# masa-ue/SVDD

Hardware: AMD Instinct MI355X
Metric: decoded sequences/sec (whole node), L=200 M=10 128-step SVDD-MC (higher is better)
Workload: dtype f32; 1 GPU; DNA enhancer SVDD-MC, batch=256/GPU, L=200, M=10, 128 steps (BASELINE.json configs[1]); dilated-CNN backbone 3.3M params + ConvGRU value net; global_batch=256, rng=philox

## Files before the change

include/svdd_hip.h:

```cpp
#ifndef SVDD_HIP_H
#define SVDD_HIP_H

#include <stdint.h>

#ifdef __cplusplus
extern "C" {
#endif

#define SVDD_VOCAB 5
#define SVDD_MASK 4
#define SVDD_MAX_M 1024

enum {
  SVDD_OK = 0,
  SVDD_E_ARG = -1,
  SVDD_E_LAUNCH = -2,
  SVDD_E_NODEVICE = -3
};

enum {
  SVDD_LAYOUT_BLV = 0,
  SVDD_LAYOUT_BVL = 1
};

// ... 99 lines not shown
int svdd_bb_layer_bwd_f32(const float* g_hn, const float* f_in, const float* tb, const float* gamma, float eps, const float* g_in,
                          const uint8_t* mask_prev, float* g_out, float* gt_out, int64_t rows, int rows_per_seq, int channels,
                          void* stream);
int svdd_gru_bidir_train_f32(const float* x, const float* wpack, const float* bpack, float* out, float* save, int n, int L,
                             void* stream);
int svdd_gru_bidir_bwd_f32(const float* grad_out, const float* out, const float* save, const float* wpack_bwd, float* dx, int n,
                           int L, void* stream);
int svdd_value_tail_f32(const float* h_fwd, const float* h_bwd, const float* w1pack, const float* b1,
                        const float* w_eff, const float* b_eff, float* out, int n, int L, int n_tasks,
                        const int32_t* count, void* stream);
int svdd_gru_set_mode(int mode);

int svdd_epilogue_ln_f32(const float* y, const float* bias, const float* f_prev, const float* tb,
                         const float* gamma, const float* beta, float* f_out, float* hn, int64_t rows,
                         int channels, int act, void* stream);

int svdd_conv1d_cl_f32(const float* x, const float* wpack, float* y, int n, int L, int cin, int cout,
                       int taps, int dilation, const float* bias, const float* f_prev, int act,
                       const float* tb, const float* gamma, const float* beta, float* hn, void* stream);
int svdd_conv1d_set_dynamic(int on);

int svdd_conv_tower_f32(const float* onehot, const float* tiles, const float* bias, float* out, int n, int L,
                        int nlayers, int residual_mask, const int32_t* count, void* stream);

int svdd_set_backbone_packing(int full);

int svdd_set_tower_version(int v);

int svdd_candidate_windows(const uint8_t* cand, const uint8_t* x, int B, int L, int M, int margin, int32_t* win,
                           int32_t* flags, void* stream);
int svdd_conv_tower_windows_f32(const float* onehot, const float* tiles, const float* bias, const int32_t* win,
                                const float* parent_out, float* out, int n, int L, int M, int nlayers,
                                int residual_mask, const int32_t* live_idx, const int32_t* count, void* stream);

int svdd_backbone_cnn_f32(const uint8_t* x, const float* table0, const float* tiles, const float* vec,
                          const float* w2, float* out, int n, int L, int nlayers, const int* dilations,
                          const int32_t* count, const int32_t* row_idx, int out_scatter, void* stream);
int svdd_backbone_cnn_save_f32(const uint8_t* x, const float* table0, const float* tiles, const float* vec, const float* w2,
                               float* out, int n, int L, int nlayers, const int* dilations, float* xhat, float* rstd,
                               unsigned long long* mask, void* stream);
int svdd_backbone_cnn_grad_f32(const float* dlogits, const float* tiles_bwd, const float* gamma, const float* w2,
                               const float* table0, const float* xhat, const float* rstd, const unsigned long long* mask,
                               float* dx, int n, int L, int nlayers, const int* dilations, void* stream);
int svdd_backbone_incr_f32(const uint8_t* x, const float* table0, const float* tiles, const float* vec, const float* w2,
                           float* out, int n, int L, int nlayers, const int* dilations, int lead, float* planes,
                           uint8_t* x_prev, int32_t* items, unsigned long long* stat, int first, int max_item, void* on_stream);
int svdd_backbone_incr2_f32(const uint8_t* x, const float* table0, const float* tiles, const float* vec, const float* w2,
                            float* out, int n, int L, int nlayers, const int* dilations, int lead, float* planes,
                            uint8_t* x_prev, int32_t* items, unsigned long long* stat, int first, int max_item,
                            int32_t* order, int32_t* order_count, void* on_stream);
int svdd_backbone_incr_set_residency(int wg_per_cu);
int svdd_backbone_set_workspace(void* ws, long long bytes);
int svdd_backbone_split_status(int* err);

enum { SVDD_PREC_F32 = 0, SVDD_PREC_F16X3 = 1, SVDD_PREC_BF16X3 = 2, SVDD_PREC_F16 = 3, SVDD_PREC_BF16 = 4 };

int svdd_backbone_cnn_lp(const uint8_t* x, const float* table0, const void* tiles, const float* vec,
                         const float* lscale, const float* w2, float* out, int n, int L, int nlayers,
                         const int* dilations, int prec, const int32_t* count, const int32_t* row_idx, int out_scatter,
                         void* stream);

int svdd_conv_tower_lp(const uint8_t* tok, const void* tiles, const float* bias, const float* inv, void* out,
                       int n, int L, int nlayers, int residual_mask, const int32_t* count, int prec, void* stream);
int svdd_conv_tower_windows_lp(const uint8_t* cand, const void* tiles, const float* bias, const float* inv,
                               const int32_t* win, const void* parent_out, void* out, int n, int L, int M,
                               int nlayers, int residual_mask, const int32_t* live_idx, const int32_t* count,
// ... 77 lines not shown
```

svdd_amd/_lib.py:

```python
import ctypes
import os
import subprocess

_HERE = os.path.dirname(os.path.abspath(__file__))
CSRC = os.path.join(_HERE, "csrc")
SO_PATH = os.environ.get("SVDD_HIP_LIB") or os.path.join(CSRC, "libsvdd_hip.so")
ABI_VERSION = 17

OK, E_ARG, E_LAUNCH, E_NODEVICE = 0, -1, -2, -3
LAYOUT_BLV, LAYOUT_BVL = 0, 1
RNG_REPLAY, RNG_PHILOX = 0, 1
SELECT_ARGMAX, SELECT_MULTINOMIAL = 0, 1
TARGET_MEAN, TARGET_LOGMEANEXP = 0, 1
EVOLVE_GLOBAL, EVOLVE_ROW = 0, 1
ATTR_GRADIENT, ATTR_TIMES_INPUT = 0, 1
PRECISIONS = {"f32": 0, "f16x3": 1, "bf16x3": 2, "f16": 3, "bf16": 4}
MAX_M = 1024

OPT_FORCE_EXACT, OPT_MSPLIT, OPT_SELECT_ONE_ROW, OPT_BACKBONE_LP_VERSION, OPT_TRUNK_GEMM_VERSION = 0, 1, 2, 3, 4
OPT_CAND_ROW_STRIDE, OPT_TRUNK_PLANES_F32, OPT_BACKBONE_SPLIT, OPT_SELECT_BATCHES = 5, 6, 7, 8


class SvddRng(ctypes.Structure):
    _fields_ = [("kind", ctypes.c_int32), ("step", ctypes.c_uint32), ("uniforms", ctypes.c_void_p),
# ... 62 lines not shown
    "svdd_trunk_attn_pool": (vp, vp, i32, i32, i32, vp, vp, vp, vp, vp, vp, i32, STREAM),
    "svdd_trunk_stem_unfold": (vp, i32, i32, vp, vp, STREAM),
    "svdd_trunk_attn_small": (vp, vp, vp, vp, i32, i32, i32, i32, i32, vp, vp, vp, STREAM),
    "svdd_trunk_windows": (vp, vp, vp, i32, i32, i32, i32, i32, i32, vp, vp, vp, vp, STREAM),
    "svdd_trunk_stem_unfold_win": (vp, i32, i32, i32, vp, vp, vp, vp, vp, STREAM),
    "svdd_trunk_attn_pool_win": (vp, vp, i32, i32, i32, i32, i32, vp, vp, vp, vp, i32, vp, vp, vp, vp, vp, vp, vp, i32, vp, vp, vp, STREAM),
    "svdd_bb_layer_fwd_f32": (vp, vp, vp, vp, vp, vp, f32, vp, vp, vp, i64, i32, i32, STREAM),
    "svdd_bb_layer_bwd_f32": (vp, vp, vp, vp, f32, vp, vp, vp, vp, i64, i32, i32, STREAM),
    "svdd_mt19937_uniform_f32": (vp, vp, i64, STREAM),
    "svdd_backbone_set_workspace": (vp, i64),
    "svdd_backbone_split_status": (pi32,),
    "svdd_backbone_cnn_save_f32": (vp, vp, vp, vp, vp, vp, i32, i32, i32, pi32, vp, vp, vp, STREAM),
    "svdd_backbone_cnn_grad_f32": (vp, vp, vp, vp, vp, vp, vp, vp, vp, i32, i32, i32, pi32, STREAM),
    "svdd_dps_probs": (vp, vp, i32, i32, vp, STREAM),
    "svdd_dps_probs_bwd": (vp, vp, vp, i32, i32, vp, vp, STREAM),
    "svdd_dps_guided_q": (vp, vp, vp, vp, f32, f32, f32, i32, i32, vp, STREAM),
    "svdd_reward_stem_f32": (vp, vp, vp, vp, i32, i32, i32, STREAM),
    "svdd_reward_stem_bwd_f32": (vp, vp, vp, i32, i32, i32, STREAM),
    "svdd_conv1d_cl_gated_f32": (vp, vp, vp, i32, i32, i32, i32, i32, i32, vp, vp, STREAM),
    "svdd_reward_tail_grad_f32": (vp, vp, vp, vp, vp, vp, vp, f32, i32, i32, vp, vp, STREAM),
    "svdd_sum_gate_f32": (vp, vp, vp, vp, i64, STREAM),
    "svdd_gru_bidir_train2_f32": (vp, vp, vp, vp, vp, vp, i32, i32, STREAM),
    "svdd_gru_bidir_bwd2_f32": (vp, vp, vp, vp, vp, vp, vp, i32, i32, STREAM),
    "svdd_classifier_propose": (vp, i32, vp, vp, f32, f32, f32, i32, i32, RNG, vp, vp, vp, STREAM),
    "svdd_elbo_mask": (vp, i32, i32, i32, f64, RNG, vp, vp, vp, vp, vp, vp, STREAM),
    "svdd_elbo_nll": (vp, i32, vp, vp, vp, i32, i32, i32, vp, vp, vp, vp, STREAM),
    "svdd_refine_remask": (vp, vp, vp, vp, vp, f32, i32, i32, RNG, vp, vp, vp, vp, vp, vp, vp),
    "svdd_value_target": (vp, vp, i32, i32, i32, i32, f32, vp, vp, vp, vp),
    "svdd_ism_mutants": (vp, vp, vp, i32, i32, i32, vp, vp, vp, vp),
    "svdd_ism_fold": (vp, vp, vp, vp, vp, vp, i32, i32, i32, i32, i32, vp, vp, vp, vp, vp),
    "svdd_evolve_apply": (vp, vp, vp, i32, i32, i32, vp, vp, vp, vp, vp, vp, vp, vp, vp, vp, vp, vp),
    "svdd_attr_path": (vp, vp, i32, vp, i32, i32, i32, i32, i32, i32, vp, vp, vp),
    "svdd_attr_fold": (vp, f32, vp, vp, vp, i32, i32, i32, i32, i32, i32, i32, vp, vp, vp, vp),
}
EXPORTS = tuple(SIGNATURES)


def build(force=False):
    import glob
    srcs = sorted(glob.glob(os.path.join(CSRC, "*.hip")) + glob.glob(os.path.join(CSRC, "*.h")) + [os.path.join(CSRC, "Makefile")])
    srcs.append(os.path.join(os.path.dirname(_HERE), "include", "svdd_hip.h"))
    if os.environ.get("SVDD_HIP_LIB"):
        return SO_PATH
    stale = not os.path.exists(SO_PATH) or os.path.getmtime(SO_PATH) < max(os.path.getmtime(f) for f in srcs)
    if force or stale:
        subprocess.check_call(["make", "-C", CSRC, "-B", "-j", str(min(8, os.cpu_count() or 1))])
    return SO_PATH


_lib = None


def lib():
    global _lib
    if _lib is not None:
        return _lib
    import torch
    if not os.path.exists(SO_PATH):
        raise SvddError(f"{SO_PATH} is missing: build it with `python -c 'import __graft_entry__ as g; g.build()'` "
                        "or `make -C svdd_amd/csrc`. There is no CPU fallback for the SVDD hot path.")
    L = ctypes.CDLL(SO_PATH)
    for name in EXPORTS:
        if not hasattr(L, name):
            raise SvddError(f"libsvdd_hip.so does not export {name}")
    if L.svdd_abi_version() != ABI_VERSION:
        raise SvddError(f"libsvdd_hip.so ABI {L.svdd_abi_version()} != binding ABI {ABI_VERSION}; rebuild")
# ... 102 lines not shown
```

svdd_amd/csrc/svdd_nets.hip:

```cpp
#include "svdd_host.h"

namespace {

typedef float f32x4 __attribute__((ext_vector_type(4)));

__device__ __forceinline__ float wave_sum(float v) {
#pragma unroll
  for (int off = 32; off > 0; off >>= 1) v += __shfl_xor(v, off, 64);
  return v;
}


constexpr int H = 64;
constexpr int HPAD = H + 4;

__device__ __forceinline__ float sigmoid_fast(float a) {
  return __builtin_amdgcn_rcpf(1.0f + __builtin_amdgcn_exp2f(-1.44269504088896f * a));
}
__device__ __forceinline__ float tanh_fast(float a) {
  return 1.0f - 2.0f * __builtin_amdgcn_rcpf(1.0f + __builtin_amdgcn_exp2f(2.88539008177793f * a));
}

template <bool BOTH>
__global__ __launch_bounds__(BOTH ? 512 : 256) void gru_bidir_kernel(const float* __restrict__ x, const float* __restrict__ wpack,
// ... 1131 lines not shown
    }
  }
  for (int e = tid; e < (TW_ROWS + 2) * TW_AP; e += 512) smem[e] = 0.0f;

  TowerCtx2 c;
  c.act = act; c.xs = xs; c.bias = a.bias;
  c.L = L; c.tile_rows = tile_rows; c.nlayers = a.nlayers; c.residual_mask = a.residual_mask;
  constexpr int CG = 4 / CT, RS = 2 * CT;
  c.cp = w % CG; c.rq = w / CG; c.j = lane & 15; c.g = lane >> 4;
  c.wsrc = a.tiles + (16 * CT * c.cp + c.j) * CH + 8 * c.g;
#pragma unroll
  for (int r = 0; r < 7; ++r) {
    const int row = 16 * (c.rq + RS * r) + c.j;
    c.apos[r] = (!SPT1 && !WIN && row < tile_rows) ? row % L : -(1 << 20);
  }
  const int nlive = ((WIN ? nt : TW_ROWS / 16) - c.rq + RS - 1) / RS;
  __syncthreads();
  tower2_dispatch<SPT1 || WIN, WIN, CT>(c, nlive);
  if (WIN) {
    for (int e = tid; e < L * 16; e += 512) {
      const int row = e >> 4, q = e & 15;
      if (row >= keep_lo && row < keep_hi)
        *reinterpret_cast<float4*>(outc + (size_t)row * TW_C + 4 * q) = *reinterpret_cast<const float4*>(act + (row - w0) * TW_AP + 4 * q);
    }
  } else {
    for (int e = tid; e < tile_rows * 16; e += 512) {
      const int row = e >> 4, q = e & 15;
      if (row0 + row < total_rows)
        *reinterpret_cast<float4*>(a.out + (row0 + row) * TW_C + 4 * q) = *reinterpret_cast<const float4*>(act + row * TW_AP + 4 * q);
    }
  }
}

__global__ __launch_bounds__(256) void candidate_windows_kernel(const uint8_t* __restrict__ cand, const uint8_t* __restrict__ x,
                                                               int n, int L, int M, int margin, int* __restrict__ win,
                                                               int* __restrict__ flags) {
  const int c = blockIdx.x * 4 + (threadIdx.x >> 6);
  if (c >= n) return;
  const int lane = threadIdx.x & 63;
  const uint8_t* cp = cand + (size_t)c * L;
  const uint8_t* xp = x + (size_t)(c / M) * L;
  int lo = 1 << 30, hi = -1;
  for (int l = lane; l < L; l += 64)
    if (cp[l] != xp[l]) { lo = min(lo, l); hi = max(hi, l); }
#pragma unroll
  for (int off = 32; off > 0; off >>= 1) { lo = min(lo, __shfl_xor(lo, off, 64)); hi = max(hi, __shfl_xor(hi, off, 64)); }
  if (lane == 0) {
    int w0 = 0, w1 = 0;
    if (hi >= 0) {
      w0 = max(0, lo - margin) & ~15;
      w1 = min((L + 15) & ~15, (hi + margin + 1 + 15) & ~15);
    }
    win[2 * c] = w0; win[2 * c + 1] = w1;
    if (flags) flags[c] = (w1 - w0) >> 4;
  }
}


struct BackboneArgs {
  const uint8_t* x;
  const float* table0;
  const float* tiles;
  const float* vec;
  const float* w2;
  float* out;
  int n, L, spt, nl;
  int dil[BB_MAXL];
  const int* count;
  const int* row_idx;
  int out_scatter;
  int auto_spt, ncu;
  SvddTilePlan plan;
  float* planes;
  int planes_P;
};

struct BackboneSave {
  float* xhat;
  float* rstd;
  unsigned long long* mask;
};

// ... 560 lines not shown
  int* toks = reinterpret_cast<int*>(rstat + ROWS);

  int item, seq;
  if (ORD) {
    if ((int)blockIdx.x >= a.order_count[a.layer - 1]) return;
    const unsigned ent = (unsigned)__builtin_amdgcn_readfirstlane(a.order[(size_t)(a.layer - 1) * a.order_stride + blockIdx.x]);
    item = (int)(ent & 0xFFFFu);
    seq = (int)(ent >> 16);
  } else {
    item = __builtin_amdgcn_readfirstlane(a.items[(size_t)(a.layer - 1) * a.n * SEG_SLOTS + blockIdx.x]);
    seq = blockIdx.x / SEG_SLOTS;
  }
  const int nown = min(item >> 8, NC);
  if (nown == 0) return;
  const int t0 = item & 255;
  const int tid = threadIdx.x, lane = tid & 63;
  const int cg = __builtin_amdgcn_readfirstlane(tid >> 6);
  const int j = lane & 15, g = lane >> 4;
  const int col0 = 32 * cg + j;
  const int L = a.L;
  const int r0 = 16 * (t0 - 1);
  const size_t pl_stride = (size_t)a.n * TW_ROWS * BB_C;
  float* pl0 = a.planes + (size_t)seq * TW_ROWS * BB_C;
  const int cl = a.layer - 1;
#define SEG_LIVE(S) ((S) <= nown + 1)

  f32x4 f[NS][2], acc[NS][2];
  if (a.layer == 1) {
    for (int e = tid; e < ROWS + 8; e += 256) {
      const int p = r0 - 4 + e;
      toks[e] = (p >= 0 && p < L) ? (int)a.x[(size_t)seq * L + p] : -1;
    }
    __syncthreads();
#pragma unroll
    for (int ct = 0; ct < 2; ++ct) {
      const int col = col0 + 16 * ct;
      const float b0 = a.vec[col];
#pragma unroll
      for (int s = 0; s < NS; ++s) {
        if (!SEG_LIVE(s)) continue;
#pragma unroll
        for (int e = 0; e < 4; ++e) {
          const int ri = 16 * s + 4 * g + e, row = r0 + ri;
          float v = b0;
#pragma unroll
          for (int t = 0; t < 9; ++t) {
            const int tk = toks[ri + t];
            if (tk >= 0) v += a.table0[(t * 5 + tk) * BB_C + col];
          }
          f[s][ct][e] = (row >= 0 && row < L) ? fmaxf(v, 0.0f) : 0.0f;
        }
      }
    }
  } else {
    const float* src = pl0 + (size_t)(a.layer - 2) * pl_stride;
#pragma unroll
    for (int s = 0; s < NS; ++s) {
      if (!SEG_LIVE(s)) continue;
#pragma unroll
      for (int ct = 0; ct < 2; ++ct)
#pragma unroll
        for (int e = 0; e < 4; ++e) {
          const int row = r0 + 16 * s + 4 * g + e;
          f[s][ct][e] = (row >= 0 && row < L) ? src[row * BB_C + col0 + 16 * ct] : 0.0f;
        }
    }
  }

  const float* vl = a.vec + (size_t)(cl + 1) * 4 * BB_C;
  {
    const float tb0 = vl[BB_C + col0], tb1 = vl[BB_C + col0 + 16];
#pragma unroll
    for (int s = 0; s < NS; ++s) {
      if (!SEG_LIVE(s)) continue;
#pragma unroll
      for (int e = 0; e < 4; ++e) {
        const float sm = group16_sum((f[s][0][e] + tb0) + (f[s][1][e] + tb1));
        if (j == 0) psum[cg * ROWS + 16 * s + 4 * g + e] = sm;
      }
    }
    __syncthreads();
    if (tid < 16 * (nown + 2))
      rstat[tid] = ((psum[tid] + psum[ROWS + tid]) + (psum[2 * ROWS + tid] + psum[3 * ROWS + tid])) * (1.0f / BB_C);
    __syncthreads();
#pragma unroll
// ... 1136 lines not shown
  void (*seg)(BackboneSegArgs) = max_item == 4 ? backbone_seg_kernel<4, true> : max_item == 2 ? backbone_seg_kernel<2, true>
                                                                                                : backbone_seg_kernel<1, true>;
  svdd_raise_lds_limit(seg, slds);
  for (int k = 1; k <= lead; ++k) {
    sa.layer = k;
    if (svdd_launch(seg, sgrid, dim3(256), slds, stream, sa) != SVDD_OK) return SVDD_E_LAUNCH;
  }
  return svdd_launch_timed(span.last(), backbone_kernel<true, false, 2>, dim3((unsigned)n), dim3(512), lds, stream, a, BackboneSave{});
}

typedef decltype(&value_tail_kernel<1>) ValueTailKernel;

extern "C" int svdd_value_tail_f32(const float* h_fwd, const float* h_bwd, const float* w1pack, const float* b1,
                                   const float* w_eff, const float* b_eff, float* out, int n, int L, int n_tasks,
                                   const int32_t* count, void* stream) {
  if (!h_fwd || !h_bwd || !w1pack || !b1 || !w_eff || !b_eff || !out || n <= 0 || L <= 0 || n_tasks < 1 || n_tasks > 4)
    return SVDD_E_ARG;
  ValueTailKernel kern;
  switch (n_tasks) {
    case 1: kern = value_tail_kernel<1>; break;
    case 2: kern = value_tail_kernel<2>; break;
    case 3: kern = value_tail_kernel<3>; break;
    default: kern = value_tail_kernel<4>; break;
  }
  SvddSpan span(SVDD_SLOT_VALUE_TAIL);
  return svdd_launch_timed(span.all(), kern, dim3((unsigned)((n + 3) / 4)), dim3(256), 0, stream, h_fwd, h_bwd, w1pack, b1, w_eff, b_eff, out,
                           n, L, count);
}

extern "C" int svdd_candidate_windows(const uint8_t* cand, const uint8_t* x, int B, int L, int M, int margin, int32_t* win,
                                      int32_t* flags, void* stream) {
  if (!cand || !x || !win || B <= 0 || L <= 0 || M <= 0 || margin < 0) return SVDD_E_ARG;
  const int n = B * M;
  return svdd_launch(candidate_windows_kernel, dim3((unsigned)((n + 3) / 4)), dim3(256), 0, stream, cand, x, n, L, M, margin, win, flags);
}

extern "C" int svdd_conv_tower_windows_f32(const float* onehot, const float* tiles, const float* bias, const int32_t* win,
                                           const float* parent_out, float* out, int n, int L, int M, int nlayers,
                                           int residual_mask, const int32_t* live_idx, const int32_t* count, void* stream) {
  if (!onehot || !tiles || !bias || !win || !parent_out || !out || n <= 0 || M <= 0 || (n % M && !live_idx) || L <= TW_ROWS / 2 ||
      L > TW_ROWS || nlayers != 5)
    return SVDD_E_ARG;
  TowerWinArgs wa{TowerArgs{onehot, tiles, bias, out, n, L, 1, nlayers, residual_mask, nullptr}, win, parent_out, M, live_idx, count};
  void (*kern)(TowerWinArgs) = conv_tower_win_kernel;
  if (g_tower_ver != 1) kern = g_tower_ver == 2 ? conv_tower2_kernel<true, true, 2> : conv_tower2_kernel<true, true, 1>;
  SvddSpan span(SVDD_SLOT_CONV_TOWER);
  return svdd_launch_timed(span.all(), kern, dim3((unsigned)n), dim3(512), svdd_lds_raised(tower2_lds_bytes()), stream, wa);
}
```

svdd_amd/diffusion.py:

```python
import contextlib
import functools
import math
import warnings
import weakref
from dataclasses import dataclass
from typing import Optional

import numpy as np
import torch
import torch.nn.functional as F
from torch import nn

from . import noise_schedule, ops
from .backbone import CNNModel


@dataclass
class Loss:
    loss: torch.Tensor
    nlls: torch.Tensor
    token_mask: torch.Tensor


@dataclass
# ... 1030 lines not shown
        pos, pos_dev = self._ism_positions(positions, x.shape[1])
        if chunk_rows is not None and int(chunk_rows) <= 0:
            raise ValueError(f"chunk_rows must be positive, got {chunk_rows}")
        if not x.dtype.is_floating_point and x.dtype != torch.bool and bool((x == self.mask_index).any()):
            raise ops.SvddError("x holds a MASK token: in-silico mutagenesis scores finished sequences (tokens 0..3)")
        x_u8, _ = self._refine_inputs(x, None)
        self._require_gpu()
        B, L = x_u8.shape
        if chunk_rows is None:
            chunk_rows = self.ISM_WAVES_PER_CHUNK * torch.cuda.get_device_properties(self.device).multi_processor_count
        Pc = max(1, min(len(pos), int(chunk_rows) // (3 * B)))
        return x_u8, pos_dev, len(pos), Pc

    class _IsmWorkspace:
        def __init__(self, B, L, Pc, dev, windowed):
            n = B * 3 * Pc
            self.cand = torch.empty(n * L, dtype=torch.uint8, device=dev)
            self.onehot = self.flags = self.live_idx = self.slot = self.count = None
            if windowed:
                self.onehot = torch.empty(n * L * 4, dtype=torch.float32, device=dev)
                self.flags, self.live_idx, self.slot = (torch.empty(n, dtype=torch.int32, device=dev) for _ in range(3))
                self.count = torch.zeros(1, dtype=torch.int32, device=dev)
            self.err = torch.zeros(1, dtype=torch.int32, device=dev)

    def _ism_route(self, pre_scorer_embedding, pre_scorer_head, reward_model, L):
        from .fused import FusedValueNet
        score_fn = self._design_scorer(pre_scorer_embedding, pre_scorer_head, reward_model)
        fn = (self.value_callable(pre_scorer_embedding, pre_scorer_head) if reward_model is None
              else self.reward_callable(reward_model))
        windowed = isinstance(fn, FusedValueNet) and fn.kernels_ok(L) and fn.candidates_ok(L, 3)
        return score_fn, (fn if windowed else None)

    def _ism_pass(self, x, pos_dev, P, Pc, score_fn, fused, ws, parent_score, live=None, ism=None, best=None):
        from . import fused as F_
        B, L = x.shape
        lp = fused is not None and fused.precision != "f32"
        if fused is not None:
            parent_out = fused.parent_tower(x)
        for p0 in range(0, P, Pc):
            pc = min(Pc, P - p0)
            n = B * 3 * pc
            cand = ws.cand[:n * L].view(B, 3 * pc, L)
            if fused is None:
                ops.ism_mutants(x, pos_dev[p0:p0 + pc], live, cand=cand, want_onehot=False, err=ws.err)
                ops.ism_fold(score_fn(cand.view(n, L)), parent_score, x, pos_dev, p0, pc, live=live, ism=ism, best=best)
                continue
            onehot = None if lp else ws.onehot[:n * L * 4].view(n, L, 4)
            ops.ism_mutants(x, pos_dev[p0:p0 + pc], live, cand=cand, onehot=onehot, want_onehot=False, err=ws.err)
            if live is None:
                win = F_.candidate_windows(cand, x)
                sc = fused.forward_candidates_from(onehot, cand, win, parent_out)
                slot = None
            else:
                flags, live_idx, slot = ws.flags[:n], ws.live_idx[:n], ws.slot[:n]
                win = F_.candidate_windows(cand, x, flags=flags)
                ops.compact_flags(flags, live_idx, slot, ws.count)
                sc = fused.forward_candidates_from(onehot, cand, win, parent_out, live_idx=live_idx, count=ws.count)
            sc = sc.reshape(n, -1)
            sc = sc.reshape(n) if sc.shape[1] == 1 else sc[:, 0].contiguous()
            ops.ism_fold(sc, parent_score, x, pos_dev, p0, pc, slot=slot, live=live, ism=ism, best=best)

    @torch.no_grad()
    def ism_scores(self, x, pre_scorer_embedding, pre_scorer_head, reward_model=None, positions=None, compare=None, chunk_rows=None):
        if compare not in self.ISM_COMPARE:
            raise ValueError(f"compare = {compare!r}: expected None, 'subtract', 'divide' or 'log2FC'")
        x_u8, pos_dev, P, Pc = self._ism_inputs(x, positions, chunk_rows)
        B, L = x_u8.shape
        score_fn, fused = self._ism_route(pre_scorer_embedding, pre_scorer_head, reward_model, L)
        ws = self._IsmWorkspace(B, L, Pc, self.device, fused is not None)
        parent_score = score_fn(x_u8)
        ism = torch.empty((B, P, 4), dtype=torch.float32, device=self.device)
        self._ism_pass(x_u8, pos_dev, P, Pc, score_fn, fused, ws, parent_score, ism=ism)
        ops.check_ism_err(ws.err)
        if compare is not None:
            ref = parent_score[:, None, None]
            ism = ism - ref if compare == "subtract" else ism / ref if compare == "divide" else torch.log2(ism / ref)
        return ism

    @torch.no_grad()
    def evolve(self, x, pre_scorer_embedding, pre_scorer_head, reward_model=None, max_iter=10, positions=None, stop="global",
               chunk_rows=None):
        if stop not in ops.EVOLVE_STOP:
            raise ValueError(f"stop = {stop!r}: expected 'global' or 'row'")
        max_iter = int(max_iter)
        if max_iter < 0:
            raise ValueError(f"max_iter must be >= 0, got {max_iter}")
        x_u8, pos_dev, P, Pc = self._ism_inputs(x, positions, chunk_rows)
        x_u8 = x_u8.clone()
# ... 523 lines not shown
```

svdd_amd/fused.py:

```python
import ctypes
import math

import torch
import torch.nn.functional as F
from torch import nn

from . import _lib
from .backbone import CNNModel
from .value_nets import ConvGRUTrunk, ConvHead


def _cl(w):
    return w.detach().unsqueeze(2).contiguous(memory_format=torch.channels_last)


def pack_gru(gru):
    H = gru.hidden_size
    assert H == 64 and gru.input_size == 64 and gru.bidirectional and gru.num_layers == 1 and gru.bias
    packs, biases = [], []
    for sfx in ("", "_reverse"):
        w_ih = getattr(gru, "weight_ih_l0" + sfx).detach().float()
        w_hh = getattr(gru, "weight_hh_l0" + sfx).detach().float()
        b_ih = getattr(gru, "bias_ih_l0" + sfx).detach().float()
        b_hh = getattr(gru, "bias_hh_l0" + sfx).detach().float()
# ... 476 lines not shown
    B, M, L = cand.shape
    n = B * M
    if out is None:
        out = torch.empty((n, L, parent_out.shape[2], 64), dtype=tiles.dtype, device=cand.device)
    _lib.call("svdd_conv_tower_windows_lp", cand, tiles, bias, inv, win, parent_out, out, n, L, M, bias.shape[0] - 1, int(residual_mask),
              live_idx, count, prec)
    return out


def gru_bidir_lp(x_nlc, wpack, bpack, inv, prec, count=None, out=None):
    assert x_nlc.is_cuda and x_nlc.is_contiguous() and x_nlc.shape[-1] == 64
    split = x_nlc.dim() == 4
    assert split or x_nlc.dtype == torch.float32
    n, L = x_nlc.shape[0], x_nlc.shape[1]
    if out is None:
        out = torch.empty((2, n, L, 64), dtype=torch.float32, device=x_nlc.device)
    _lib.call("svdd_gru_bidir_lp", None if split else x_nlc, x_nlc if split else None, wpack, bpack, inv, out, n, L, count, prec)
    return out


def value_tail_lp(h, w1pack, b1f, w_eff, b_eff, inv, prec, count=None, out=None):
    _, n, L, _ = h.shape
    T = w_eff.shape[1]
    if out is None:
        out = torch.empty((n, T), dtype=torch.float32, device=h.device)
    assert out.is_contiguous() and out.shape == (n, T) and out.dtype == torch.float32
    _lib.call("svdd_value_tail_lp", h[0], h[1], w1pack, b1f, w_eff, b_eff, float(inv), out, n, L, T, count, prec)
    return out


TOWER_WINDOW_MARGIN = 27


def candidate_windows(cand, x, margin=TOWER_WINDOW_MARGIN, flags=None):
    assert cand.is_cuda and cand.dtype == torch.uint8 and cand.is_contiguous() and x.dtype == torch.uint8 and x.is_contiguous()
    B, M, L = cand.shape
    win = torch.empty((B * M, 2), dtype=torch.int32, device=cand.device)
    _lib.call("svdd_candidate_windows", cand, x, B, L, M, margin, win, flags)
    return win


def conv_tower_windows(onehot, win, parent_out, M, tiles, bias, residual_mask, live_idx=None, count=None, out=None):
    assert onehot.is_cuda and onehot.dtype == torch.float32 and onehot.is_contiguous() and onehot.shape[2] == 4
    n, L, _ = onehot.shape
    assert parent_out.is_contiguous() and parent_out.shape == (n // M, L, 64) and win.shape == (n, 2)
    if out is None:
        out = torch.empty((n, L, 64), dtype=torch.float32, device=onehot.device)
    else:
        assert live_idx is not None and count is not None and out.is_contiguous() and out.shape[1:] == (L, 64)
        n = out.shape[0]
    _lib.call("svdd_conv_tower_windows_f32", onehot, tiles, bias, win, parent_out, out, n, L, M, bias.shape[0] - 1, int(residual_mask),
              live_idx, count)
    return out


def epilogue_ln(y, bias=None, f_prev=None, tb=None, gamma=None, beta=None, act=ACT_RELU_THEN_ADD, want_norm=True,
                want_sum=True):
    C = bias.numel() if bias is not None else gamma.numel()
    rows = y.numel() // C
    f = torch.empty_like(y) if want_sum else None
    hn = torch.empty_like(y) if want_norm else None
    assert y.dtype == torch.float32 and (f if f is not None else hn).stride() == y.stride()
    _lib.call("svdd_epilogue_ln_f32", y, bias, f_prev, tb, gamma, beta, f, hn, rows, C, int(act))
    return f, hn


class FusedValueNet(nn.Module):

    def __init__(self, embedding: ConvGRUTrunk, head: ConvHead):
        super().__init__()
        blocks = embedding.conv_tower.blocks
# ... 22 lines not shown
        stem = blocks[0].conv
        self.tower_ok = (tuple(stem.weight.shape) == (64, 4, 15) and 1 <= len(ws) <= 8 and
                         all(tuple(w.shape) == (64, 64, 5) for w in folded_ws) and
                         all(blk.conv.dilation[0] == 1 for blk in blocks[1:]))
        if self.tower_ok:
            self.tw_tiles = nn.Parameter(pack_tower(stem.weight, folded_ws), requires_grad=False)
            self.tw_bias = nn.Parameter(torch.stack([stem.bias.detach()] + [b.detach() for b in bs]).contiguous(),
                                        requires_grad=False)
            self.tw_resmask = sum(1 << k for k, r in enumerate(self.residual) if r)
        self.use_fused_tower = True
        gt = embedding.gru_tower
        wpack, bpack = pack_gru(gt.gru)
        self.register_buffer("wpack", wpack)
        self.register_buffer("bpack", bpack)
        d1, d2 = gt.ffn.dense1, gt.ffn.dense2
        self.ln_w = nn.Parameter(d1.norm.layer.weight.detach().clone(), requires_grad=False)
        self.ln_b = nn.Parameter(d1.norm.layer.bias.detach().clone(), requires_grad=False)
        self.w1 = nn.Parameter(d1.linear.weight.detach().clone(), requires_grad=False)
        self.b1 = nn.Parameter(d1.linear.bias.detach().clone(), requires_grad=False)
        hw = head.channel_transform.conv.layer
        wh, bh = hw.weight.detach()[:, :, 0].double(), hw.bias.detach().double()
        w2, b2 = d2.linear.weight.detach().double(), d2.linear.bias.detach().double()
        self.w_eff = nn.Parameter((wh @ w2).float().t().contiguous(), requires_grad=False)
        self.b_eff = nn.Parameter((wh @ b2 + bh).float(), requires_grad=False)
        self.tail_ok = tuple(self.w1.shape) == (128, 64) and self.w_eff.shape[1] <= 4
        if self.tail_ok:
            wp, bf = pack_tail(self.w1, self.b1, self.ln_w, self.ln_b)
            self.w1pack = nn.Parameter(wp, requires_grad=False)
            self.b1f = nn.Parameter(bf, requires_grad=False)
        self.use_fused_tail = True
        self.share_parent_tower = True
        self.split_gru_rounds = True
        self.sort_live_by_window = True
        self.precision = "f32"
        self._gru_mod = (gt.gru,)
        self._stem_w_raw = stem.weight.detach()
        self._folded_ws = [w.detach() for w in folded_ws]
        self._lp = {}
        self._grad_packs = None
        self.gru_off_chain = True
        self._ln_eps = d1.norm.layer.eps
        self.keep_grad_pass = False
        self.last_grad_pass = None

    def lp_ok(self, L):
        return self.precision != "f32" and self.tower_ok and self.tail_ok and L <= 208

    def _lp_pack(self):
        pk = self._lp.get(self.precision)
        if pk is None:
            dev = self.tw_bias.device
            tiles, tinv = pack_tower_lp(self._stem_w_raw.to(dev), [w.to(dev) for w in self._folded_ws], self.precision)
            gw, gb, ginv = pack_gru_lp(self._gru_mod[0], self.precision)
            tw, tb1, tail_inv = pack_tail_lp(self.w1, self.b1, self.ln_w, self.ln_b, self.precision)
            pk = dict(prec=_lib.PRECISIONS[self.precision], tiles=tiles.to(dev), tinv=tinv.to(dev), gw=gw.to(dev),
                      gb=gb.to(dev), ginv=ginv.to(dev), tw=tw.to(dev), tb1=tb1.to(dev), tail_inv=tail_inv)
            self._lp[self.precision] = pk
        return pk

    def forward_tokens(self, tok, count=None, out=None):
        from . import ops
        if self.precision != "f32":
            pk = self._lp_pack()
            seq = conv_tower_lp(tok.contiguous(), pk["tiles"], self.tw_bias, pk["tinv"], self.tw_resmask, pk["prec"], count)
            return self._after_tower_lp(seq, pk, count, out)
        seq = conv_tower(ops.transform_samples(tok.contiguous()), self.tw_tiles, self.tw_bias, self.tw_resmask, count)
# ... 41 lines not shown
        gout = torch.empty_like(out)
        w_eff0 = self.w_eff[:, 0].contiguous()
        dxg = torch.empty((2, n, L, 64), dtype=torch.float32, device=dev)
        if self.gru_off_chain:
            _lib.call("svdd_gru_bidir_train2_f32", fs[-1], self.wpack, self.bpack, gates, out, save, n, L)
        else:
            _lib.call("svdd_gru_bidir_train_f32", fs[-1], self.wpack, self.bpack, out, save, n, L)
        _lib.call("svdd_reward_tail_grad_f32", out[0], out[1], self.w1, self.b1, self.ln_w, self.ln_b, w_eff0, float(self._ln_eps), n, L,
                  gout[0], gout[1])
        g = dxg[1]
        if self.gru_off_chain:
            _lib.call("svdd_gru_bidir_bwd2_f32", gout, out, save, gru_bwd, gates, fs[-1], g, n, L)
        else:
            dxd = torch.empty_like(out)
            _lib.call("svdd_gru_bidir_bwd_f32", gout, out, save, gru_bwd, dxd, n, L)
            _lib.call("svdd_sum_gate_f32", dxd[0], dxd[1], fs[-1], g, n * L * 64)
        bufs = [gout[1], dxg[0]]
        for k in range(len(packs_t) - 1, -1, -1):
            y = bufs[k & 1]
            _lib.call("svdd_conv1d_cl_gated_f32", g, packs_t[k], y, n, L, 64, 64, 5, 1, g if self.residual[k] else None, fs[k])
            g = y
        dx = torch.empty((n, L, 4), dtype=torch.float32, device=dev)
        _lib.call("svdd_reward_stem_bwd_f32", g, w_stem, dx, n, L, self._stem_w_raw.shape[2])
        if self.keep_grad_pass:
            self.last_grad_pass = {"fs": fs, "out": out, "g_tail": gout[0], "grad": dx}
        return dx

    def kernels_ok(self, L):
        return self.use_fused_tower and self.tower_ok and self.use_fused_tail and self.tail_ok and L <= 208

    def candidate_scores_compact(self, onehot, cand, x, ws):
        from . import ops
        B, M, L = cand.shape
        win = candidate_windows(cand, x, flags=ws.flags)
        split = self._gru_split(B * M) if (self.precision == "f32" and getattr(ws, "late", False)) else 0
        if split:
            ops.compact_by_key(ws.flags, ws.live_idx, ws.slot, ws.count3, split=split)
        else:
            (ops.compact_by_key if self.sort_live_by_window else ops.compact_flags)(ws.flags, ws.live_idx, ws.slot, ws.count)
        if getattr(ws, "n_win_rows", None) is not None:
            ws.n_win_rows += (win[:, 1] - win[:, 0]).sum()
        lp = self.precision != "f32"
        if ws.parent_out is None or ws.parent_out_lp != self.precision:
            xp = x[:1].contiguous() if getattr(ws, "prior_rows_identical", False) else x
            if lp:
                pk = self._lp_pack()
                po = conv_tower_lp(xp, pk["tiles"], self.tw_bias, pk["tinv"], self.tw_resmask, pk["prec"])
            else:
                po = conv_tower(ops.transform_samples(xp), self.tw_tiles, self.tw_bias, self.tw_resmask)
            ws.parent_out = po if xp is x else po.expand(B, *po.shape[1:]).contiguous()
            ws.prior_rows_identical = False
            ws.parent_out_lp = self.precision
        if lp:
            pk = self._lp_pack()
            ws.seq = conv_tower_windows_lp(cand, win, ws.parent_out, pk["tiles"], self.tw_bias, pk["tinv"], self.tw_resmask,
                                           pk["prec"], live_idx=ws.live_idx, count=ws.count)
            return self._after_tower_lp(ws.seq, pk, ws.count)[:, :, 0]
        if split:
            return self._windows_gru_tail_split(onehot, win, ws, B * M, L, M, split)
        ws.seq = conv_tower_windows(onehot, win, ws.parent_out, M, self.tw_tiles, self.tw_bias, self.tw_resmask,
                                    live_idx=ws.live_idx, count=ws.count)
        return self._after_tower(ws.seq, B * M, L, ws.count)[:, :, 0]

    GRU_ROUND_ROWS = None

    def gru_round_rows(self):
        if self.GRU_ROUND_ROWS is not None:
# ... 42 lines not shown

    def _after_tower_lp(self, seq, pk, count=None, out=None):
        h = gru_bidir_lp(seq, pk["gw"], pk["gb"], pk["ginv"], pk["prec"], count=count)
        return value_tail_lp(h, pk["tw"], pk["tb1"], self.w_eff, self.b_eff, pk["tail_inv"], pk["prec"], count=count, out=out)[:, :, None]

    def forward(self, x):
        if x.shape[1] == self.in_channels and x.shape[2] != self.in_channels:
            x = x.transpose(1, 2)
        n, L, C = x.shape
        if self.lp_ok(L) and x.is_cuda:
            tok = torch.where(x.sum(dim=2) == 0, 4, x.argmax(dim=2)).to(torch.uint8)
            return self.forward_tokens(tok)
        if self.use_fused_tower and self.tower_ok and L <= 208 and x.is_cuda:
            seq = conv_tower(x.contiguous(), self.tw_tiles, self.tw_bias, self.tw_resmask)
            return self._after_tower(seq, n, L)
        f = x.contiguous().view(n, 1, L, C).permute(0, 3, 1, 2)
        f, _ = epilogue_ln(F.conv2d(f, self.stem_w, None, padding=(0, self.stem_pad)), self.stem_b, want_norm=False)
        hip_conv = self.use_hip_conv and L in (200, 50) and n * L >= 192 * 200
        for w, b, wp, pad, res in zip(self.ws, self.bs, self.wpacks, self.pads, self.residual):
            if hip_conv and wp.numel():
                seq = f.permute(0, 2, 3, 1).reshape(n, L, 64)
                f = conv1d_cl(seq, wp, 64, 5, 1, bias=b, f_prev=seq if res else None, act=ACT_ADD_THEN_RELU)
                f = f.view(n, 1, L, 64).permute(0, 3, 1, 2)
            else:
                y = F.conv2d(f, w, None, padding=(0, pad))
                f, _ = epilogue_ln(y, b, f if res else None, act=ACT_ADD_THEN_RELU, want_norm=False)
        seq = f.permute(0, 2, 3, 1).reshape(n, L, f.shape[1])
        return self._after_tower(seq.contiguous(), n, L)

    def candidates_ok(self, L, M):
        return (self.use_fused_tower and self.tower_ok and self.share_parent_tower and M > 1 and 104 < L <= 208 and
                self.tw_bias.shape[0] == 6)

    def forward_candidates(self, onehot, cand, x):
        from . import ops
        B, M, L = cand.shape
        if self.lp_ok(L):
            pk = self._lp_pack()
            parent_out = conv_tower_lp(x, pk["tiles"], self.tw_bias, pk["tinv"], self.tw_resmask, pk["prec"])
            win = candidate_windows(cand, x)
            seq = conv_tower_windows_lp(cand, win, parent_out, pk["tiles"], self.tw_bias, pk["tinv"], self.tw_resmask, pk["prec"])
            return self._after_tower_lp(seq, pk)
        parent_out = conv_tower(ops.transform_samples(x), self.tw_tiles, self.tw_bias, self.tw_resmask)
        win = candidate_windows(cand, x)
        seq = conv_tower_windows(onehot, win, parent_out, M, self.tw_tiles, self.tw_bias, self.tw_resmask)
        return self._after_tower(seq, B * M, L)

    def parent_tower(self, x):
        from . import ops
        if self.lp_ok(x.shape[1]):
            pk = self._lp_pack()
            return conv_tower_lp(x, pk["tiles"], self.tw_bias, pk["tinv"], self.tw_resmask, pk["prec"])
        return conv_tower(ops.transform_samples(x), self.tw_tiles, self.tw_bias, self.tw_resmask)

    def forward_candidates_from(self, onehot, cand, win, parent_out, live_idx=None, count=None):
        B, M, L = cand.shape
        if self.lp_ok(L):
            pk = self._lp_pack()
            seq = conv_tower_windows_lp(cand, win, parent_out, pk["tiles"], self.tw_bias, pk["tinv"], self.tw_resmask, pk["prec"],
                                        live_idx=live_idx, count=count)
            return self._after_tower_lp(seq, pk, count)
        seq = conv_tower_windows(onehot, win, parent_out, M, self.tw_tiles, self.tw_bias, self.tw_resmask, live_idx=live_idx, count=count)
        return self._after_tower(seq, B * M, L, count)

    def _after_tower(self, seq, n, L, count=None, out=None):
        h = gru_bidir(seq, self.wpack, self.bpack, count)
        if self.use_fused_tail and self.tail_ok:
            return value_tail(h, self.w1pack, self.b1f, self.w_eff, self.b_eff, count, out=out)[:, :, None]
        assert count is None and out is None, "compacted batches need the fused tail kernel"
        _, hn = epilogue_ln(h[0], None, h[1], None, self.ln_w, self.ln_b, act=ACT_NONE, want_sum=False)
        z = F.relu(F.linear(hn, self.w1, self.b1))
        return ((z @ self.w_eff).mean(dim=1) + self.b_eff)[:, :, None]


class FusedBackbone(nn.Module):

    def __init__(self, cnn: CNNModel):
# ... 120 lines not shown
```

Before: 768.2 sequences/s.

## Use unaligned tight candidate windows and stage backbone first-layer table lookups in LDS

Adds a tight variant of the candidate-window kernel that starts the recompute window at the exact lower bound instead of rounding down to 16. Only the window length is padded to a multiple of 16, so the windowed conv tower recomputes fewer rows per candidate in f32 mode, and callers switch to it through a new windows_of helper. Separately, the incremental backbone first layer now builds its embedding-table sums cooperatively into a shared image, one channel per thread, with branch-free gathers, then reads fragments from that image. The risks are misaligned window starts that downstream tower kernels may not expect, plus extra LDS traffic and an added barrier.

```diff
diff --git a/include/svdd_hip.h b/include/svdd_hip.h
--- a/include/svdd_hip.h
+++ b/include/svdd_hip.h
@@ -155,6 +155,9 @@
 int svdd_conv_tower_windows_f32(const float* onehot, const float* tiles, const float* bias, const int32_t* win,
                                 const float* parent_out, float* out, int n, int L, int M, int nlayers,
                                 int residual_mask, const int32_t* live_idx, const int32_t* count, void* stream);
+
+int svdd_candidate_windows_tight(const uint8_t* cand, const uint8_t* x, int B, int L, int M, int margin, int32_t* win,
+                                 int32_t* flags, void* on_stream);
 
 int svdd_backbone_cnn_f32(const uint8_t* x, const float* table0, const float* tiles, const float* vec,
                           const float* w2, float* out, int n, int L, int nlayers, const int* dilations,
diff --git a/svdd_amd/_lib.py b/svdd_amd/_lib.py
--- a/svdd_amd/_lib.py
+++ b/svdd_amd/_lib.py
@@ -118,6 +118,7 @@
     "svdd_evolve_apply": (vp, vp, vp, i32, i32, i32, vp, vp, vp, vp, vp, vp, vp, vp, vp, vp, vp, vp),
     "svdd_attr_path": (vp, vp, i32, vp, i32, i32, i32, i32, i32, i32, vp, vp, vp),
     "svdd_attr_fold": (vp, f32, vp, vp, vp, i32, i32, i32, i32, i32, i32, i32, vp, vp, vp, vp),
+    "svdd_candidate_windows_tight": (vp, vp, i32, i32, i32, i32, vp, vp, vp),
 }
 EXPORTS = tuple(SIGNATURES)
 
diff --git a/svdd_amd/csrc/svdd_nets.hip b/svdd_amd/csrc/svdd_nets.hip
--- a/svdd_amd/csrc/svdd_nets.hip
+++ b/svdd_amd/csrc/svdd_nets.hip
@@ -1187,6 +1187,7 @@
   }
 }
 
+template <bool TIGHT>
 __global__ __launch_bounds__(256) void candidate_windows_kernel(const uint8_t* __restrict__ cand, const uint8_t* __restrict__ x,
                                                                int n, int L, int M, int margin, int* __restrict__ win,
                                                                int* __restrict__ flags) {
@@ -1202,7 +1203,10 @@
   for (int off = 32; off > 0; off >>= 1) { lo = min(lo, __shfl_xor(lo, off, 64)); hi = max(hi, __shfl_xor(hi, off, 64)); }
   if (lane == 0) {
     int w0 = 0, w1 = 0;
-    if (hi >= 0) {
+    if (hi >= 0 && TIGHT) {
+      w0 = max(0, lo - margin);
+      w1 = w0 + ((min(L, hi + margin + 1) - w0 + 15) & ~15);
+    } else if (hi >= 0) {
       w0 = max(0, lo - margin) & ~15;
       w1 = min((L + 15) & ~15, (hi + margin + 1 + 15) & ~15);
     }
@@ -1829,25 +1833,33 @@
       toks[e] = (p >= 0 && p < L) ? (int)a.x[(size_t)seq * L + p] : -1;
     }
     __syncthreads();
-#pragma unroll
-    for (int ct = 0; ct < 2; ++ct) {
-      const int col = col0 + 16 * ct;
-      const float b0 = a.vec[col];
-#pragma unroll
-      for (int s = 0; s < NS; ++s) {
-        if (!SEG_LIVE(s)) continue;
-#pragma unroll
-        for (int e = 0; e < 4; ++e) {
-          const int ri = 16 * s + 4 * g + e, row = r0 + ri;
-          float v = b0;
-#pragma unroll
-          for (int t = 0; t < 9; ++t) {
-            const int tk = toks[ri + t];
-            if (tk >= 0) v += a.table0[(t * 5 + tk) * BB_C + col];
-          }
-          f[s][ct][e] = (row >= 0 && row < L) ? fmaxf(v, 0.0f) : 0.0f;
-        }
-      }
+    {
+      const int c = tid & (BB_C - 1);
+      const float b0 = a.vec[c];
+#pragma unroll 4
+      for (int ri = tid >> 7; ri < 16 * (nown + 2); ri += 2) {
+        int tk[9];
+        float tv[9];
+#pragma unroll
+        for (int t = 0; t < 9; ++t) {
+          tk[t] = toks[ri + t];
+          tv[t] = a.table0[(unsigned)((t * 5 + max(tk[t], 0)) * BB_C + c)];
+        }
+        float v = b0;
+#pragma unroll
+        for (int t = 0; t < 9; ++t) v = tk[t] >= 0 ? v + tv[t] : v;
+        const int row = r0 + ri;
+        img[ri * BB_AP + c] = (row >= 0 && row < L) ? fmaxf(v, 0.0f) : 0.0f;
+      }
+    }
+    __syncthreads();
+#pragma unroll
+    for (int s = 0; s < NS; ++s) {
+      if (!SEG_LIVE(s)) continue;
+#pragma unroll
+      for (int ct = 0; ct < 2; ++ct)
+#pragma unroll
+        for (int e = 0; e < 4; ++e) f[s][ct][e] = img[(16 * s + 4 * g + e) * BB_AP + col0 + 16 * ct];
     }
   } else {
     const float* src = pl0 + (size_t)(a.layer - 2) * pl_stride;
@@ -3050,7 +3062,16 @@
                                       int32_t* flags, void* stream) {
   if (!cand || !x || !win || B <= 0 || L <= 0 || M <= 0 || margin < 0) return SVDD_E_ARG;
   const int n = B * M;
-  return svdd_launch(candidate_windows_kernel, dim3((unsigned)((n + 3) / 4)), dim3(256), 0, stream, cand, x, n, L, M, margin, win, flags);
+  return svdd_launch(candidate_windows_kernel<false>, dim3((unsigned)((n + 3) / 4)), dim3(256), 0, stream, cand, x, n, L, M, margin, win, flags);
+}
+
+extern "C" int svdd_candidate_windows_tight(const uint8_t* cand, const uint8_t* x, int B, int L, int M, int margin, int32_t* win,
+                                            int32_t* flags, void* on_stream) {
+  if (!cand || !x || !win || B <= 0 || L <= 0 || M <= 0 || margin < 0 || margin > (1 << 20) ||
+      (long long)B * M > 0x7fffffffLL)
+    return SVDD_E_ARG;
+  const int n = B * M;
+  return svdd_launch(candidate_windows_kernel<true>, dim3((unsigned)((n + 3) / 4)), dim3(256), 0, on_stream, cand, x, n, L, M, margin, win, flags);
 }
 
 extern "C" int svdd_conv_tower_windows_f32(const float* onehot, const float* tiles, const float* bias, const int32_t* win,
diff --git a/svdd_amd/diffusion.py b/svdd_amd/diffusion.py
--- a/svdd_amd/diffusion.py
+++ b/svdd_amd/diffusion.py
@@ -1086,7 +1086,6 @@
         return score_fn, (fn if windowed else None)
 
     def _ism_pass(self, x, pos_dev, P, Pc, score_fn, fused, ws, parent_score, live=None, ism=None, best=None):
-        from . import fused as F_
         B, L = x.shape
         lp = fused is not None and fused.precision != "f32"
         if fused is not None:
@@ -1102,12 +1101,12 @@
             onehot = None if lp else ws.onehot[:n * L * 4].view(n, L, 4)
             ops.ism_mutants(x, pos_dev[p0:p0 + pc], live, cand=cand, onehot=onehot, want_onehot=False, err=ws.err)
             if live is None:
-                win = F_.candidate_windows(cand, x)
+                win = fused.windows_of(cand, x)
                 sc = fused.forward_candidates_from(onehot, cand, win, parent_out)
                 slot = None
             else:
                 flags, live_idx, slot = ws.flags[:n], ws.live_idx[:n], ws.slot[:n]
-                win = F_.candidate_windows(cand, x, flags=flags)
+                win = fused.windows_of(cand, x, flags=flags)
                 ops.compact_flags(flags, live_idx, slot, ws.count)
                 sc = fused.forward_candidates_from(onehot, cand, win, parent_out, live_idx=live_idx, count=ws.count)
             sc = sc.reshape(n, -1)
diff --git a/svdd_amd/fused.py b/svdd_amd/fused.py
--- a/svdd_amd/fused.py
+++ b/svdd_amd/fused.py
@@ -532,11 +532,15 @@
 TOWER_WINDOW_MARGIN = 27
 
 
-def candidate_windows(cand, x, margin=TOWER_WINDOW_MARGIN, flags=None):
+def candidate_windows(cand, x, margin=TOWER_WINDOW_MARGIN, flags=None, tight=False):
     assert cand.is_cuda and cand.dtype == torch.uint8 and cand.is_contiguous() and x.dtype == torch.uint8 and x.is_contiguous()
     B, M, L = cand.shape
     win = torch.empty((B * M, 2), dtype=torch.int32, device=cand.device)
-    _lib.call("svdd_candidate_windows", cand, x, B, L, M, margin, win, flags)
+    if tight:
+        _lib.call("svdd_candidate_windows_tight", cand, x, B, L, M, margin, win, flags,
+                  ctypes.c_void_p(torch.cuda.current_stream().cuda_stream))
+    else:
+        _lib.call("svdd_candidate_windows", cand, x, B, L, M, margin, win, flags)
     return win
 
 
@@ -625,6 +629,7 @@
         self.share_parent_tower = True
         self.split_gru_rounds = True
         self.sort_live_by_window = True
+        self.tight_windows = True
         self.precision = "f32"
         self._gru_mod = (gt.gru,)
         self._stem_w_raw = stem.weight.detach()
@@ -732,7 +737,7 @@
     def candidate_scores_compact(self, onehot, cand, x, ws):
         from . import ops
         B, M, L = cand.shape
-        win = candidate_windows(cand, x, flags=ws.flags)
+        win = self.windows_of(cand, x, flags=ws.flags)
         split = self._gru_split(B * M) if (self.precision == "f32" and getattr(ws, "late", False)) else 0
         if split:
             ops.compact_by_key(ws.flags, ws.live_idx, ws.slot, ws.count3, split=split)
@@ -841,6 +846,9 @@
         return (self.use_fused_tower and self.tower_ok and self.share_parent_tower and M > 1 and 104 < L <= 208 and
                 self.tw_bias.shape[0] == 6)
 
+    def windows_of(self, cand, x, flags=None):
+        return candidate_windows(cand, x, flags=flags, tight=self.tight_windows and self.precision == "f32")
+
     def forward_candidates(self, onehot, cand, x):
         from . import ops
         B, M, L = cand.shape
@@ -851,7 +859,7 @@
             seq = conv_tower_windows_lp(cand, win, parent_out, pk["tiles"], self.tw_bias, pk["tinv"], self.tw_resmask, pk["prec"])
             return self._after_tower_lp(seq, pk)
         parent_out = conv_tower(ops.transform_samples(x), self.tw_tiles, self.tw_bias, self.tw_resmask)
-        win = candidate_windows(cand, x)
+        win = self.windows_of(cand, x)
         seq = conv_tower_windows(onehot, win, parent_out, M, self.tw_tiles, self.tw_bias, self.tw_resmask)
         return self._after_tower(seq, B * M, L)
 
```

Measured after the change: 780.4 sequences/s (median of 6 runs). +1.6%, better.
